# pmelchior/proxmin

Measured on AMD Instinct MI355X. Metric: NMF iterations/sec at Y=16384x16384, K=64, higher is better.
Workload: dtype f16x2r (fp16 split MFMA, fp32 accumulate: the residual from the high x high product + an exact K x K correction, two-term gradients; exact fp32's error class)

## Files before the change

proxmin_amd/csrc/k_gfix.hip:

```cpp
#include "pmx_common.h"

constexpr int GFIX_PARTS = 128;

struct GfixArgs {
    const float* X[2];
    int64_t rows[2];
    int K;
    const float* absmax;
    float* part;
    float* Q;
    float* out[2];
    int ld;
    int want[2];
    const DevStatus* status;
    long long* prof;
};
#define GFIX_STAMP(i) do { if (a.prof != nullptr && blockIdx.x == 0 && blockIdx.y == 0 && threadIdx.x == 0) a.prof[i] = wall_clock64(); } while (0)

typedef _Float16 gf16x8 __attribute__((ext_vector_type(8)));

__device__ __forceinline__ float gfix_scale(const float* absmax, int f, float* red) {
    float m = 0.f;
    for (int i = threadIdx.x; i < 256; i += blockDim.x) m = fmaxf(m, absmax[f * 256 + i]);
#pragma unroll
    for (int o = 32; o > 0; o >>= 1) m = fmaxf(m, __shfl_xor(m, o));
    if ((threadIdx.x & 63) == 0) red[threadIdx.x >> 6] = m;
    __syncthreads();
    float mx = red[0];
    for (int i = 1; i < (int)(blockDim.x >> 6); ++i) mx = fmaxf(mx, red[i]);
    int q = 0;
    (void)frexpf(mx, &q);
    return ldexpf(1.f, mx > 0.f ? 14 - q : 0);
}

template <int KT, int W>
__device__ __forceinline__ void gfix_gram_wave(const GfixArgs& a, int f, float* red) {
    constexpr int K = 32 * KT, TPW = KT * KT / 4, NB = KT == 2 ? 8 : 4;
    const int lane = threadIdx.x & 63, l31 = lane & 31, hi = lane >> 5;
    const int64_t rows = a.rows[f];
    const int64_t per = 16 * ((rows + 16 * GFIX_PARTS - 1) / (16 * GFIX_PARTS));
    const int64_t r0 = (int64_t)blockIdx.x * per, r1 = r0 + per < rows ? r0 + per : rows;
    const float* X = a.X[f] + 32 * 0 + l31;
    f32x16 acc0[TPW], accr[TPW];
#pragma unroll
    for (int t = 0; t < TPW; ++t)
#pragma unroll
        for (int i = 0; i < 16; ++i) { acc0[t][i] = 0.f; accr[t][i] = 0.f; }
// ... 145 lines not shown
        const float* p = a.part + (int64_t)f * GFIX_PARTS * n + (int64_t)(q * 32) * n + e;
        float v[32];
#pragma unroll
        for (int i = 0; i < 32; ++i) v[i] = p[(int64_t)i * n];
#pragma unroll
        for (int i = 0; i < 32; ++i) s += (double)v[i];
    }
    const int base = threadIdx.x & 60;
    double tot = __shfl(s, base);
#pragma unroll
    for (int i = 1; i < 4; ++i) tot += __shfl(s, base + i);
    if (e < n && q == 0) a.Q[(int64_t)f * n + e] = (float)tot;
    GFIX_STAMP(5);
}

template <int KT>
__global__ __launch_bounds__(KT == 4 ? 512 : 256) void k_gfix_apply(GfixArgs a) {
    constexpr int K = 32 * KT, LDQ = K + 8;
    constexpr int NT = KT == 4 ? 512 : 256, NW = NT / 64;
    extern __shared__ _Float16 qpl[];
    __shared__ float red[8];
    if (chain_halted(a.status)) return;
    const int f = blockIdx.y;
    if (!a.want[f]) return;
    const int tid = threadIdx.x, lane = tid & 63, w = tid >> 6, l31 = lane & 31, hi = lane >> 5;
    const int64_t rows = a.rows[f];
    const float* X = a.X[f];
    float* out = a.out[f];
    const int64_t ntask = (rows + 31) / 32 * KT, stride = (int64_t)gridDim.x * NW;
    if ((int64_t)blockIdx.x * NW >= ntask) return;
    GFIX_STAMP(6);
    f32x4 x[K / 16][2];
#define GFIX_LOAD_X(t_)                                                                                                   \
    {                                                                                                                     \
        const int64_t row_ = ((t_) / KT) * 32 + l31;                                                                      \
        const f32x4* xr = reinterpret_cast<const f32x4*>(X + (row_ < rows ? row_ : 0) * K + 8 * hi);                       \
        _Pragma("unroll") for (int ks = 0; ks < K / 16; ++ks) { x[ks][0] = xr[4 * ks]; x[ks][1] = xr[4 * ks + 1]; }       \
    }
    const int64_t task0 = (int64_t)blockIdx.x * NW + w;
    if (task0 < ntask) GFIX_LOAD_X(task0)
    constexpr int TPK = NT / K, NBLK = K / 8 / TPK;
    const int kcol = tid % K, kb0 = tid / K;
    float tq[2][NBLK][8];
    {
        const float* src = a.Q + (int64_t)(1 - f) * 2 * K * K;
#pragma unroll
        for (int m = 0; m < 2; ++m)
#pragma unroll
            for (int i = 0; i < NBLK; ++i)
#pragma unroll
                for (int e = 0; e < 8; ++e) tq[m][i][e] = src[(size_t)m * K * K + (size_t)(8 * (kb0 + TPK * i) + e) * K + kcol];
    }
    float mx[2] = {0.f, 0.f};
#pragma unroll
    for (int m = 0; m < 2; ++m)
// ... 1 lines not shown
        for (int i = 0; i < NBLK; ++i)
#pragma unroll
            for (int e = 0; e < 8; ++e) mx[m] = fmaxf(mx[m], fabsf(tq[m][i][e]));
#pragma unroll
    for (int o = 32; o > 0; o >>= 1) { mx[0] = fmaxf(mx[0], __shfl_xor(mx[0], o)); mx[1] = fmaxf(mx[1], __shfl_xor(mx[1], o)); }
    __shared__ float redq[2][NW];
    if (lane == 0) { redq[0][w] = mx[0]; redq[1][w] = mx[1]; }
    const float sc = gfix_scale(a.absmax, f, red);
    GFIX_STAMP(7);
    float sq[2];
#pragma unroll
    for (int m = 0; m < 2; ++m) {
        float v = redq[m][0];
#pragma unroll
        for (int i = 1; i < NW; ++i) v = fmaxf(v, redq[m][i]);
        int q = 0;
        (void)frexpf(v, &q);
        sq[m] = ldexpf(1.f, v > 0.f ? 14 - q : 0);
    }
#pragma unroll
    for (int m = 0; m < 2; ++m) {
        _Float16* ph = qpl + (size_t)((1 - m) * 2) * K * LDQ + (size_t)kcol * LDQ;
        _Float16* pl = ph + (size_t)K * LDQ;
#pragma unroll
        for (int i = 0; i < NBLK; ++i) {
            gf16x8 h8, l8;
#pragma unroll
            for (int e = 0; e < 8; ++e) {
                const float v = tq[m][i][e] * sq[m];
                const _Float16 h = (_Float16)v;
                h8[e] = h;
                l8[e] = (_Float16)(v - (float)h);
            }
            *reinterpret_cast<gf16x8*>(ph + 8 * (kb0 + TPK * i)) = h8;
            *reinterpret_cast<gf16x8*>(pl + 8 * (kb0 + TPK * i)) = l8;
        }
    }
    __syncthreads();
    GFIX_STAMP(8);
    for (int64_t task = (int64_t)blockIdx.x * NW + w; task < ntask; task += stride) {
        const int64_t rt = task / KT;
        const int c = (int)(task % KT);
        const bool live = rt * 32 + l31 < rows;
        if (task != task0) GFIX_LOAD_X(task)
        f32x16 acc1, acc2;
#pragma unroll
        for (int i = 0; i < 16; ++i) { acc1[i] = 0.f; acc2[i] = 0.f; }
        const _Float16* qb = qpl + (size_t)(32 * c + l31) * LDQ + 8 * hi;
#pragma unroll
        for (int ks = 0; ks < K / 16; ++ks) {
            gf16x8 xh, xl, xm;
#pragma unroll
            for (int e = 0; e < 8; ++e) {
                const float v = (live ? x[ks][e >> 2][e & 3] : 0.f) * sc;
                const _Float16 h = (_Float16)v;
                const float r1 = v - (float)h;
                const _Float16 l = (_Float16)r1;
                xh[e] = h; xl[e] = l; xm[e] = (_Float16)(r1 - (float)l);
            }
            const gf16x8 qrh = *reinterpret_cast<const gf16x8*>(qb + 16 * ks);
            const gf16x8 qrl = *reinterpret_cast<const gf16x8*>(qb + (size_t)K * LDQ + 16 * ks);
            const gf16x8 q0h = *reinterpret_cast<const gf16x8*>(qb + (size_t)2 * K * LDQ + 16 * ks);
            const gf16x8 q0l = *reinterpret_cast<const gf16x8*>(qb + (size_t)3 * K * LDQ + 16 * ks);
            acc1 = __builtin_amdgcn_mfma_f32_32x32x16_f16(xl, qrh, acc1, 0, 0, 0);
            acc2 = __builtin_amdgcn_mfma_f32_32x32x16_f16(xm, q0h, acc2, 0, 0, 0);
            acc1 = __builtin_amdgcn_mfma_f32_32x32x16_f16(xh, qrl, acc1, 0, 0, 0);
            acc2 = __builtin_amdgcn_mfma_f32_32x32x16_f16(xl, q0l, acc2, 0, 0, 0);
            acc1 = __builtin_amdgcn_mfma_f32_32x32x16_f16(xh, qrh, acc1, 0, 0, 0);
            acc2 = __builtin_amdgcn_mfma_f32_32x32x16_f16(xl, q0h, acc2, 0, 0, 0);
        }
        const float u1 = 1.f / (sc * sq[1]), u2 = 1.f / (sc * sq[0]);
#pragma unroll
        for (int i = 0; i < 16; ++i) {
            const int64_t r = rt * 32 + (i & 3) + 8 * (i >> 2) + 4 * hi;
            if (r < rows) out[r * a.ld + 32 * c + l31] = acc1[i] * u1 + acc2[i] * u2;
        }
        GFIX_STAMP(9);
    }
#undef GFIX_LOAD_X
    GFIX_STAMP(10);
}

static hipError_t launch_gfix(const GfixArgs& a, hipStream_t s) {
    const int n = 2 * a.K * a.K;
    const size_t lds = (size_t)4 * a.K * (a.K + 8) * sizeof(_Float16);
    const int64_t rmax = a.rows[0] > a.rows[1] ? a.rows[0] : a.rows[1];
    const int nw = a.K == 128 ? 8 : 4;
    unsigned nb = (unsigned)(((rmax + 31) / 32 * (a.K / 32) + nw - 1) / nw);
    if (nb > (a.K == 128 ? 128u : 256u)) nb = a.K == 128 ? 128 : 256;
    if (a.K == 64) {
        hipError_t e = hipFuncSetAttribute((const void*)k_gfix_apply<2>, hipFuncAttributeMaxDynamicSharedMemorySize, (int)lds);
        if (e != hipSuccess) return e;
        hipLaunchKernelGGL(k_gfix_gram<2>, dim3(GFIX_PARTS, 2), dim3(256), 0, s, a);
        hipLaunchKernelGGL(k_gfix_reduce, dim3((n * 4 + 255) / 256, 2), dim3(256), 0, s, a);
        hipLaunchKernelGGL(k_gfix_apply<2>, dim3(nb, 2), dim3(256), lds, s, a);
    } else if (a.K == 128) {
        hipError_t e = hipFuncSetAttribute((const void*)k_gfix_apply<4>, hipFuncAttributeMaxDynamicSharedMemorySize, (int)lds);
        if (e != hipSuccess) return e;
        e = hipFuncSetAttribute((const void*)k_gfix_gram<4>, hipFuncAttributeMaxDynamicSharedMemorySize, 64 * 1024);
        if (e != hipSuccess) return e;
        hipLaunchKernelGGL(k_gfix_gram<4>, dim3(GFIX_PARTS, 2), dim3(256), 64 * 1024, s, a);
        hipLaunchKernelGGL(k_gfix_reduce, dim3((n * 4 + 255) / 256, 2), dim3(256), 0, s, a);
        hipLaunchKernelGGL(k_gfix_apply<4>, dim3(nb, 2), dim3(512), lds, s, a);
    } else return hipErrorInvalidValue;
    return hipGetLastError();
}
```

proxmin_amd/csrc/k_update.hip:

```cpp
#include "pmx_common.h"

template <int CTRL>
__device__ __forceinline__ float dpp_f(float v) {
    return __builtin_bit_cast(float, __builtin_amdgcn_update_dpp(0, __builtin_bit_cast(int, v), CTRL, 0xf, 0xf, true));
}
template <int CTRL>
__device__ __forceinline__ double dpp_d(double v) {
    const unsigned long long u = __builtin_bit_cast(unsigned long long, v);
    const unsigned lo = (unsigned)__builtin_amdgcn_update_dpp(0, (int)(unsigned)u, CTRL, 0xf, 0xf, true);
    const unsigned hi = (unsigned)__builtin_amdgcn_update_dpp(0, (int)(unsigned)(u >> 32), CTRL, 0xf, 0xf, true);
    return __builtin_bit_cast(double, ((unsigned long long)hi << 32) | lo);
}
constexpr int DPP_XOR1 = 0xB1, DPP_XOR2 = 0x4E, DPP_HALF_MIRROR = 0x141, DPP_MIRROR = 0x140;
constexpr int SWZ_XOR16 = (0x10 << 10) | 0x1f;

constexpr int SWZ_XOR8 = (0x08 << 10) | 0x1f, SWZ_XOR4 = (0x04 << 10) | 0x1f;
__device__ __forceinline__ float row_sum32(float v) {
    v += __builtin_bit_cast(float, __builtin_amdgcn_ds_swizzle(__builtin_bit_cast(int, v), SWZ_XOR16));
    v += __builtin_bit_cast(float, __builtin_amdgcn_ds_swizzle(__builtin_bit_cast(int, v), SWZ_XOR8));
    v += __builtin_bit_cast(float, __builtin_amdgcn_ds_swizzle(__builtin_bit_cast(int, v), SWZ_XOR4));
    v += dpp_f<DPP_XOR2>(v);
    v += dpp_f<DPP_XOR1>(v);
    return v;
}
// ... 1323 lines not shown
        for (unsigned spins = 1; (gb_load(&b->gen[g][0]) >> 1) < e; ++spins) {
            __builtin_amdgcn_s_sleep(4);
            if ((spins & 1023u) == 0 && wall_clock64() - t0 > 10000000) {
                st->tail_fault = 2;
                st->reason = HALT_ERROR;
                __threadfence();
                st->halt = 1;
                break;
            }
        }
    }
    __syncthreads();
}

constexpr int TAIL_NT = 4;
struct TailArgs {
    MomentArgs m;
    ProxSeq prox[2];
    double e_rel[2];
    int prox_max_iter;
    double* colpart;
    float* absmax_out;
    AlphaArgs al;
    int decide_check;
    GridBar* bar;
    int slots[2];
    long long* prof;
    int prof_fine;
};
template <int NC>
__global__ __launch_bounds__(EW_THREADS) void k_ada_tail(TailArgs a) {
    __shared__ double scratch[4 * TAIL_NT * EW_WAVES];
    __shared__ double dbuf[EW_BLOCKS + 8];
    __shared__ unsigned s_word;
    extern __shared__ float lds[];
    static_assert(EW_BLOCKS == 2 * MAXK, "the step-size phase gives one (block, component) to each workgroup");
    DevStatus* st = a.m.status;
    if (chain_halted(st)) return;
    const int tid = threadIdx.x, l32 = tid & 31;
    const int K = a.m.K;
    GridBar* bar = a.bar;
    unsigned ep = bar->epoch[0];
    int nstamp = 0;
    auto stamp = [&]() { if (a.prof != nullptr && blockIdx.x == 0 && tid == 0) a.prof[nstamp++] = wall_clock64(); };
    stamp();
    if (tid == 0) gb_arrive(bar, ep + 1, true);
    const int64_t hw = ((int64_t)blockIdx.x * EW_THREADS + tid) >> 5;
    const int64_t nhw = ((int64_t)EW_BLOCKS * EW_THREADS) >> 5;
    const int nslot = a.slots[0] + a.slots[1];
    float* Lx = lds;
    float* Lz = lds + (size_t)nslot * NC * EW_THREADS;
    float* Lp = lds + (size_t)2 * nslot * NC * EW_THREADS;
    auto slot = [&](int j, int i, int c) { return ((size_t)((j ? a.slots[0] : 0) + i) * NC + c) * EW_THREADS + tid; };
    bool ok[NC];
#pragma unroll
    for (int c = 0; c < NC; ++c) ok[c] = l32 + 32 * c < K;
    const MomentScalars ms = moment_scalars(a.m);
    const bool any_prox = a.m.has_prox[0] || a.m.has_prox[1];

    float g_pre[NC], x_pre[NC];
    const bool pre = a.slots[0] > 0 && hw < a.m.rows[0];
    if (pre) {
        load_grad<NC>(g_pre, ok, a.m.slab[0], a.m.rows[0], K, hw, l32);
#pragma unroll
        for (int c = 0; c < NC; ++c) x_pre[c] = ok[c] ? a.m.X[0][hw * K + l32 + 32 * c] : 0.f;
    }
    float alpha0[NC], alpha1[NC];
#pragma unroll
    for (int c = 0; c < NC; ++c) {
        alpha0[c] = ok[c] ? st->alpha[0][l32 + 32 * c] : 0.f;
        alpha1[c] = ok[c] ? st->alpha[1][l32 + 32 * c] : 0.f;
    }
    const int last_tau0 = st->last_tau[0], last_tau1 = st->last_tau[1];
    {
        if (tid == 0) s_word = gb_wait(bar, ep + 1, 200000);
        __syncthreads();
        if (s_word & 1u) {
            if (blockIdx.x == 0 && tid == 0) {
                st->tail_fault = 1;
                st->reason = HALT_ERROR;
                __threadfence();
                st->halt = 1;
            }
            return;
        }
        ep += 1;
    }
    stamp();
// ... 3 lines not shown
        float alpha[NC];
#pragma unroll
        for (int c = 0; c < NC; ++c) alpha[c] = j ? alpha1[c] : alpha0[c];
        float maxpsi = -1.f;
        for (int i = 0; i < a.slots[j]; ++i) {
            const int64_t r = hw + (int64_t)i * nhw;
            if (r >= rows) break;
            float g[NC], xo[NC];
            if (j == 0 && i == 0 && pre) {
#pragma unroll
                for (int c = 0; c < NC; ++c) { g[c] = g_pre[c]; xo[c] = x_pre[c]; }
            } else {
                load_grad<NC>(g, ok, a.m.slab[j], rows, K, r, l32);
#pragma unroll
                for (int c = 0; c < NC; ++c) xo[c] = ok[c] ? a.m.X[j][r * K + l32 + 32 * c] : 0.f;
            }
#pragma unroll
            for (int c = 0; c < NC; ++c) {
                if (!ok[c]) continue;
                const int64_t e = r * K + l32 + 32 * c;
                float psi;
                const float xn = moment_elem(a.m, ms, j, e, g[c], alpha[c], xo[c], psi);
                if (a.m.check_convergence) a.m.Xp[j][e] = xo[c];
                Lx[slot(j, i, c)] = xn;
                Lp[slot(j, i, c)] = psi;
                maxpsi = nanmaxf(maxpsi, psi);
            }
        }
        if (j) mpsi1 = maxpsi; else mpsi0 = maxpsi;
    }
// ... 861 lines not shown
    do {                                                                                                           \
        if ((K) <= 32) hipLaunchKernelGGL((KERNEL<1, NT>), grid, dim3(EW_THREADS), 0, stream, args);                \
        else if ((K) <= 64) hipLaunchKernelGGL((KERNEL<2, NT>), grid, dim3(EW_THREADS), 0, stream, args);           \
        else hipLaunchKernelGGL((KERNEL<4, NT>), grid, dim3(EW_THREADS), 0, stream, args);                          \
    } while (0)
void launch_ada_sub(const SubArgs& a, hipStream_t s) {
    if (a.nt == 1) DISPATCH_NC_NT(a.K, 1, k_ada_sub, dim3(EW_BLOCKS, 2), s, a);
    else if (a.nt == 4) DISPATCH_NC_NT(a.K, 4, k_ada_sub, dim3(EW_BLOCKS, 2), s, a);
    else DISPATCH_NC_NT(a.K, SUB_NT_MAX, k_ada_sub, dim3(EW_BLOCKS, 2), s, a);
}
void launch_ada_finish(const FinishArgs& a, hipStream_t s) { DISPATCH_NC(a.s.K, k_ada_finish, dim3(EW_BLOCKS, 2), s, a); }
void launch_ada_decide(const AdaDecideArgs& a, hipStream_t s) { hipLaunchKernelGGL(k_ada_decide, dim3(1), dim3(EW_THREADS), 0, s, a); }
static size_t ada_tail_lds_bytes(const TailArgs& a) {
    const int NC = a.m.K <= 32 ? 1 : (a.m.K <= 64 ? 2 : 4);
    const size_t arr = (size_t)(a.slots[0] + a.slots[1]) * NC * EW_THREADS * sizeof(float);
    return 2 * arr + std::max(arr, (size_t)(EW_THREADS / 32) * MAXK * sizeof(float));
}
constexpr size_t ADA_TAIL_LDS_MAX = 160 * 1024 - 6 * 1024;
template <int NC>
static hipError_t launch_ada_tail_t(const TailArgs& a, hipStream_t s) {
    const size_t lds = ada_tail_lds_bytes(a);
    hipError_t e = hipFuncSetAttribute((const void*)k_ada_tail<NC>, hipFuncAttributeMaxDynamicSharedMemorySize, (int)lds);
    if (e != hipSuccess) return e;
    hipLaunchKernelGGL(k_ada_tail<NC>, dim3(EW_BLOCKS), dim3(EW_THREADS), lds, s, a);
    return hipGetLastError();
}
hipError_t launch_ada_tail(const TailArgs& a, hipStream_t s) {
    if (a.m.K <= 32) return launch_ada_tail_t<1>(a, s);
    if (a.m.K <= 64) return launch_ada_tail_t<2>(a, s);
    return launch_ada_tail_t<4>(a, s);
}
// ... 8 lines not shown
```

proxmin_amd/csrc/pmx_api.hip:

```cpp
#include <stdarg.h>
#include <stdio.h>
#include <string.h>
#include <math.h>
#include <vector>
#include <string>
#include <algorithm>
#include <mutex>

#include <fcntl.h>
#include <sys/file.h>
#include <unistd.h>
#include <dlfcn.h>
#include <link.h>
#include "pmx_common.h"
#include "chain_link.h"
#include "k_grad.hip"
#include "k_grad_bf16.hip"
#include "k_grad_k128.hip"
#include "k_grad_f16_k32.hip"
#include "k_grad_f32pc.hip"
#include "k_update.hip"
#include "k_gram.hip"
#include "k_gfix.hip"
#include "k_small_f64.hip"
#include "k_grad_f64.hip"
#include "k_big_f64.hip"

static thread_local char g_err[512] = "";
void pmx_set_error(const char* fmt, ...) {
    va_list ap;
    va_start(ap, fmt);
    vsnprintf(g_err, sizeof(g_err), fmt, ap);
    va_end(ap);
}
#define FAIL(code, ...)            \
    do {                           \
        pmx_set_error(__VA_ARGS__); \
        return (code);             \
// ... 68 lines not shown
    bool use_bf16 = false;
    bool use_f16 = false;
    bool k128 = false;
    bool k32f16 = false;
    bool f32pc = false;
    bool f16_fell_back = false;
    bool f16_scales = false;
    float rangeRatio = 65536.f;
    int rangeFaults = 0;
    int f16_r3 = 0;
    float* fixPart = nullptr;
    float* fixQ = nullptr;
    float* fixSlab[2] = {nullptr, nullptr};
    long long* fixProf = nullptr;
    bool fix_on = false;
    bool k1_sync_check = false;
    int ncu = 0;
    _Float16* A16[2] = {nullptr, nullptr};
    float* absmax = nullptr;
    float ymax = 0.f;
    float wmax = 1.f;
    bool absmax_by_finish = false;
    bool gram_by_update = false;
    bool bsd_decide_pending = false;
    BsdmmDecideArgs bsd_decide{};
    bool gram_fresh[2] = {false, false};
    bool gram_in_update = true;
    bool fold_in_k1 = true;
    K1GramFold k1_fold{};
    bool decide_pending = false;
// ... 457 lines not shown
    }
    for (int a = 0; a < 6; ++a) ms[a] = cnt[a] ? sum[a] / cnt[a] : 0.0;
    *iterations = cnt[0];
    return PMX_OK;
}

extern "C" int pmx_k1_info(pmx_ctx* c, int info[8]) {
    if (!c || !info) FAIL(PMX_E_INVALID, "NULL argument");
    info[0] = c->f64big ? 13 : c->f64 ? 7 : c->k32f16 ? (c->f16_r3 ? 10 : 8) : c->use_small ? 4 : (c->k128 ? (c->f16_r3 == 2 && !c->W && c->fixPart ? 12 : 5) : (c->use_f16 && !c->f16_fell_back ? (c->f16_r3 && !c->W ? (c->f16_r3 == 2 && c->fixPart ? 11 : 9) : 2) : (c->use_bf16 ? 1 : (c->f32pc ? 6 : 0))));
    info[1] = c->chainL;
    info[2] = c->nSlabA;
    info[3] = c->nSlabS;
    info[4] = c->plan.gridX;
    info[5] = c->plan.gridY;
    info[6] = c->plan.RP;
    info[7] = c->chainFaults + 1000 * c->tailFaults + (c->tail_fused ? 1000000 : 0) + 10000000 * std::min(c->rangeFaults, 9);
    return PMX_OK;
}

extern "C" int pmx_k1_frame(pmx_ctx* c, int64_t frame[3]) {
    if (!c || !frame) FAIL(PMX_E_INVALID, "NULL argument");
    frame[0] = c->f64 ? c->M : c->Mk;
    frame[1] = c->f64 ? c->N : c->Nk;
    frame[2] = c->f64 ? c->K : c->Kk;
    return PMX_OK;
}

extern "C" int pmx_ctx_sync(pmx_ctx* c) {
    if (!c) FAIL(PMX_E_INVALID, "ctx is NULL");
    HIP_CHECK(hipStreamSynchronize(c->stream));
    return PMX_OK;
// ... 306 lines not shown
    c->nSlabA = c->plan.nSlabA;
    float* big = nullptr;
    int rc = dallocT(c, &big, (size_t)c->nSlabA * c->Mk * c->Kk, false);
    if (rc != PMX_OK) return rc;
    c->slab[0] = big;
    return PMX_OK;
}
static int one_iteration_per_call(pmx_ctx* c) {
    c->k1_sync_check = true;
    return chain_disable(c);
}
static int k1_leave_f16(pmx_ctx* c) {
    c->mode = PMX_MODE_F32;
    select_k1(c, c->Mk, c->Nk, c->ncu);
    c->fix_on = false;
    if (c->k1_sync_check) {
        c->chainL = 0;
        c->nSlabA = c->plan.nSlabA;
    }
    c->chainFlags = nullptr;
    c->chainSeq = 0;
    c->slab[0] = c->slab[1] = nullptr;
    c->lossPart = nullptr;
    int rc = PMX_OK;
    if (c->chainL > 0) rc = dallocT(c, &c->chainFlags, (size_t)(c->plan.gridX * c->plan.gridY / c->chainL) * c->plan.RP * 4);
    if (rc == PMX_OK) rc = dallocT(c, &c->slab[0], (size_t)c->nSlabA * c->Mk * c->Kk, false);
    if (rc == PMX_OK) rc = dallocT(c, &c->slab[1], (size_t)c->plan.nSlabS * c->Nk * c->Kk, false);
    if (rc == PMX_OK) rc = dallocT(c, &c->lossPart, (size_t)2 * c->plan.gridX * c->plan.gridY);
    c->rangeFaults += 1;
    return rc;
// ... 68 lines not shown
    if (timed) HIP_CHECK(hipEventRecord(c->ev[c->ev_used], c->stream));
    HIP_CHECK(launch_small_front(c->plan, g, e, c->stream));
    c->nloss = c->plan.gridX * c->plan.gridY;
    if (timed) {
        HIP_CHECK(hipEventRecord(c->ev[c->ev_used + 1], c->stream));
        c->ev_used += 2;
    }
    return PMX_OK;
}

static int k1_prio_for(const pmx_ctx* c, int kk) {
    if (c->k1_prio != -999) return c->k1_prio;
    return kk == 64 ? 0 : 1;
}

static int enqueue_gfix(pmx_ctx* c, const float* A, const float* St, int doA, int doS, hipStream_t stream) {
    GfixArgs f{};
    f.X[0] = A; f.X[1] = St;
    f.rows[0] = c->M; f.rows[1] = c->N;
    f.K = (int)c->Kk;
    f.absmax = c->absmax;
    f.part = c->fixPart; f.Q = c->fixQ;
    f.out[0] = c->fixSlab[0]; f.out[1] = c->fixSlab[1];
    f.ld = (int)c->Kk;
    f.want[0] = (doA & 1) != 0; f.want[1] = doS != 0;
    f.status = c->dstatus;
    f.prof = c->fixProf;
    HIP_CHECK(launch_gfix(f, stream));
    return PMX_OK;
}

static int enqueue_grad_once(pmx_ctx* c, const float* A, const float* St, int doA, int doS, bool absmax_fresh) {
    if (c->host_grad) return PMX_OK;
    if (c->Kk != c->K) {
        PadArgs pa{};
        pa.src[0] = A; pa.src[1] = St;
        pa.dst[0] = c->Xk[0]; pa.dst[1] = c->Xk[1];
        pa.rows[0] = c->M; pa.rows[1] = c->N;
        pa.K = (int)c->K; pa.Kk = (int)c->Kk;
        pa.status = c->dstatus;
        launch_pad_factors(pa, c->stream);
        A = c->Xk[0]; St = c->Xk[1];
    }
    const int64_t Kq = c->Kk;
    bool fix_pending = false;
    const bool timed = c->timing && (c->timing_seq++ % (unsigned)c->timing_stride) == 0 && c->ev_used + 2 <= c->ev.size();
    if (c->k128) {
// ... 110 lines not shown
                HIP_CHECK(hipMemsetAsync(c->chainFlags, 0, (size_t)(c->plan.gridX * c->plan.gridY / c->chainL) * c->plan.RP * 4 * sizeof(unsigned), c->stream));
                c->chainSeq = 0;
            }
            GradArgs gc = g;
            gc.chainL = c->chainL; gc.chainFlags = c->chainFlags; gc.chainBase = (++c->chainSeq) * 64u; gc.wstatus = c->dstatus;
            gc.chainInject = c->hook_inject_k1 > 0 && (int)c->chainSeq == c->hook_inject_k1;
            HIP_CHECK(grad_launch_f32pc(c->plan, gc, c->stream));
        } else
        HIP_CHECK(c->use_small ? grad_launch_small(c->plan, g, c->stream) : (c->f32pc ? grad_launch_f32pc(c->plan, g, c->stream) : grad_launch_f32(c->plan, g, c->stream)));
        c->nloss = c->plan.gridX * c->plan.gridY;
    }
    if (timed) {
        HIP_CHECK(hipEventRecord(c->ev[c->ev_used + 1], c->stream));
        c->ev_used += 2;
    }
    if ((doA & 1) || doS) c->fix_on = fix_pending;
    if (fix_pending) { const int rcf = enqueue_gfix(c, A, St, doA, doS, c->stream); if (rcf != PMX_OK) return rcf; }
    return PMX_OK;
}

static int enqueue_grad(pmx_ctx* c, const float* A, const float* St, int doA, int doS, bool absmax_fresh = false) {
    int rc = enqueue_grad_once(c, A, St, doA, doS, absmax_fresh);
    if (rc != PMX_OK || !c->k1_sync_check || !c->f16_scales || c->host_grad || !(doA | doS)) return rc;
    rc = read_status(c);
    if (rc != PMX_OK) return rc;
    if (c->hstatus->k1_fault != 4) return PMX_OK;
    int again = 0;
    rc = chain_fault_fallback(c, &again);
    if (rc != PMX_OK) return rc;
    return enqueue_grad_once(c, A, St, doA, doS, false);
}

static SlabRef slab_ref(pmx_ctx* c, int j) {
    SlabRef s;
    s.stride = c->rowsK[j] * c->Kk;
    s.ld = (int)c->Kk;
    if (c->host_grad) {
        s.base = c->G[j];
        s.n = 1;
        s.ld = (int)c->K;
        return s;
    }
    s.base = c->slab[j];
    s.n = j == 0 ? c->nSlabA : c->nSlabS;
    if (c->fix_on) s.extra = c->fixSlab[j];
// ... 1283 lines not shown
        m.slab[1].base = c->ssplit ? c->comm_out : c->comm;
        m.slab[1].n = 1; m.slab[1].ld = (int)c->K; m.slab[1].extra = nullptr;
    }
    m.K = (int)c->K;
    m.status = c->dstatus;
    m.partials = c->partials;
    m.scheme = p.scheme;
    m.it = it;
    m.b1t = b1t; m.b1prev = b1prev; m.b2 = p.b2; m.eps = p.eps; m.p = p.p;
    m.check_convergence = p.check_convergence;
    launch_ada_moment(m, c->stream);
    HIP_CHECK(hipGetLastError());
    return PMX_OK;
}

static int ada_enqueue_tail_fused(pmx_ctx* c, int it, double b1t, double b1prev) {
    const pmx_adaprox_params& p = c->ada;
    TailArgs t{};
    MomentArgs& m = t.m;
    for (int j = 0; j < 2; ++j) {
        m.X[j] = s_view(c, j, c->X[j]); m.Xp[j] = s_view(c, j, c->Xp[j]);
        m.Mm[j] = s_view(c, j, c->Mm[j]); m.Vv[j] = s_view(c, j, c->Vv[j]);
        m.Vh[j] = p.warm_vhat ? s_view(c, j, c->Vh[j]) : nullptr;
        m.Psi[j] = nullptr;
        m.slab[j] = slab_ref(c, j);
        m.rows[j] = upd_rows(c, j);
        m.has_prox[j] = p.prox[j].n > 0;
        t.prox[j] = to_dev(p.prox[j]);
        t.e_rel[j] = p.e_rel[j];
        t.slots[j] = (int)((upd_rows(c, j) + 8191) / 8192);
// ... 5 lines not shown
    m.scheme = p.scheme;
    m.it = it;
    m.b1t = b1t; m.b1prev = b1prev; m.b2 = p.b2; m.eps = p.eps; m.p = p.p;
    m.check_convergence = p.check_convergence;
    t.prox_max_iter = p.prox_max_iter;
    t.colpart = c->colpart;
    t.absmax_out = c->f16_scales ? c->absmax : nullptr;
    t.al = alpha_args(c);
    t.al.use_fixed = p.use_fixed_steps;
    t.al.fixed[0] = (float)p.fixed_alpha[0];
    t.al.fixed[1] = (float)p.fixed_alpha[1];
    t.decide_check = c->comm ? 0 : 1;
    t.bar = c->gridbar;
    t.prof = c->tailprof;
    t.prof_fine = getenv("PMX_TAIL_PROF") && atoi(getenv("PMX_TAIL_PROF")) == 2;
    const char* lockfile = c->hook_tail_lockfile.empty() ? nullptr : c->hook_tail_lockfile.c_str();
    int lockfd = -1;
    if (lockfile) {
        lockfd = open(lockfile, O_CREAT | O_RDWR, 0600);
        if (lockfd < 0) FAIL(PMX_E_STATE, "PMX_TAIL_LOCKFILE: cannot open %s", lockfile);
        HIP_CHECK(hipStreamSynchronize(c->stream));
        if (flock(lockfd, LOCK_EX) != 0) { close(lockfd); FAIL(PMX_E_STATE, "PMX_TAIL_LOCKFILE: flock failed"); }
    }
    hipError_t le = launch_ada_tail(t, c->stream);
    if (lockfd >= 0) {
        hipError_t se = hipStreamSynchronize(c->stream);
        flock(lockfd, LOCK_UN);
        close(lockfd);
        HIP_CHECK(se);
    }
// ... 123 lines not shown
            if (rc != PMX_OK) return rc;
            if (c->hstatus->halt && c->hstatus->reason == HALT_ERROR) FAIL(PMX_E_HIP, "%s", chain_error_text(c));
        }
        fill_result(c, res, it0);
        return PMX_OK;
    }
    int done = 0;
    int tails = 0;
    while (done < n_iter && !c->hstatus->stopped) {
        const int chunk = std::min(n_iter - done, c->tail_fused ? 64 : 16);
        const int nsub = any_prox ? std::max(1, std::min(c->nsub_guess, p.prox_max_iter)) : 0;
        if (c->sub_nt != 1) c->sub_nt = nsub <= 4 ? 4 : SUB_NT_MAX;
        for (int i = 0; i < chunk; ++i) {
            const int gi = done + i;
            if (c->tail_fused) {
                rc = enqueue_grad(c, c->X[0], c->X[1], 1, 1, tails > 0);
                if (rc == PMX_OK) rc = ada_enqueue_tail_fused(c, it0 + gi, b1[gi], gi == 0 ? b1_prev : b1[gi - 1]);
                ++tails;
                if (rc != PMX_OK) return rc;
                continue;
            }
            rc = ada_enqueue_head(c, it0 + gi, b1[gi], gi == 0 ? b1_prev : b1[gi - 1], tails > 0);
            if (rc != PMX_OK) return rc;
            rc = ada_enqueue_tail(c, ada_enqueue_subs(c, 0, nsub));
            ++tails;
            if (rc != PMX_OK) return rc;
        }
        rc = read_status(c);
        if (rc != PMX_OK) return rc;
        const int nsub_enq = nsub > 0 ? ((nsub + c->sub_nt - 1) / c->sub_nt) * c->sub_nt : 0;
        int t_enq = nsub_enq;
// ... 17 lines not shown
            if (c->hstatus->it_done > it_before) t_enq = nsub_enq;
        }
        done = c->hstatus->it_done - it0;
        {
            int again = 0;
            rc = chain_fault_fallback(c, &again);
            if (rc != PMX_OK) return rc;
            if (again) { tails = 0; continue; }
        }
        if (any_prox) c->nsub_guess = std::max(2, std::max(c->hstatus->last_tau[0], c->hstatus->last_tau[1]));
        if (c->hstatus->halt && c->hstatus->reason == HALT_ERROR) FAIL(PMX_E_HIP, "%s", chain_error_text(c));
    }
    if (c->tailprof && c->tail_fused) {
        long long h[16];
        HIP_CHECK(hipMemcpy(h, c->tailprof, sizeof(h), hipMemcpyDeviceToHost));
        static const char* nm[] = {"census", "moment", "B1", "maxpsi", "sub", "B2", "judge+replay", "finish", "B3", "decide"};
        static const char* nf[] = {"census", "moment", "B1", "maxpsi", "passesA", "sumsA", "passesS", "sumsS", "(end)", "B2", "judge+replay", "finish", "B3", "decide"};
        const bool fine = getenv("PMX_TAIL_PROF") && atoi(getenv("PMX_TAIL_PROF")) == 2;
        const int np = fine ? 14 : 10;
        fprintf(stderr, "[tailprof] us:");
        for (int i = 0; i < np; ++i) fprintf(stderr, " %s=%.2f", fine ? nf[i] : nm[i], (double)(h[i + 1] - h[i]) / 100.0);
        fprintf(stderr, " total=%.2f\n", (double)(h[np] - h[0]) / 100.0);
    }
    fill_result(c, res, it0);
    return PMX_OK;
}

extern "C" int pmx_adaprox_set_alpha(pmx_ctx* c, const float* alpha) {
    REJECT_F64(c);
    if (!c || !alpha) FAIL(PMX_E_INVALID, "NULL argument");
    if (c->algo != ALG_ADAPROX || c->ada.use_fixed_steps != 2) FAIL(PMX_E_STATE, "pmx_adaprox_begin with use_fixed_steps = 2 has not been called");
    HIP_CHECK(hipSetDevice(c->device));
    HIP_CHECK(hipMemcpyAsync(&c->dstatus->alpha[0][0], alpha, sizeof(float) * c->K, hipMemcpyHostToDevice, c->stream));
    HIP_CHECK(hipMemcpyAsync(&c->dstatus->alpha[1][0], alpha + c->K, sizeof(float) * c->K, hipMemcpyHostToDevice, c->stream));
// ... 837 lines not shown
```

proxmin_amd/engine.py:

```python
from __future__ import annotations

import ctypes as C
import logging
import os

import numpy as np

from . import _lib

logger = logging.getLogger("proxmin")
_noticed = set()


def _notice(key, msg):
    if key not in _noticed:
        _noticed.add(key)
        logger.info(msg)


LIBRARY_DEFAULT_MODE = "f16x2r"
_DEFAULT_MODE = os.environ.get("PMX_MODE", LIBRARY_DEFAULT_MODE)
assert _DEFAULT_MODE in ("f32", "bf16x3", "f16x2", "f16x2r"), "PMX_MODE must be one of f32, bf16x3, f16x2, f16x2r"


# ... 226 lines not shown
        return {k: ms[i] for i, k in enumerate(self.PHASES)}, n.value

    def time_grad(self, do_A=True, do_S=True, reps=10):
        ms = C.c_double()
        _lib.check(self.lib.pmx_time_grad(self.h, int(do_A), int(do_S), int(reps), C.byref(ms)))
        return ms.value

    def k1_info(self):
        v = (C.c_int * 8)()
        _lib.check(self.lib.pmx_k1_info(self.h, v))
        keys = ("kernel", "chain", "slabs_A", "slabs_S", "row_regions", "col_regions", "panels_per_region", "chain_faults")
        d = dict(zip(keys, list(v)))
        d["kernel"] = ("k_grad_f32", "k_grad_bf16", "k_grad_f16_v8", "k_grad_f16_v9", "k_grad_small", "k_grad_f16_k128", "k_grad_f32_pc", "k64_front", "k_grad_f16_k32", "k_grad_f16_v8_r3", "k_grad_f16_k32_r3", "k_grad_f16_v8_hh", "k_grad_f16_k128_hh", "k64_grad_pass")[d["kernel"]]
        v7 = d.pop("chain_faults")
        d["chain_faults"], d["tail_faults"], d["tail_fused"] = v7 % 1000, (v7 // 1000) % 1000, bool((v7 // 1000000) % 10)
        d["range_faults"] = v7 // 10000000
        fr = (C.c_int64 * 3)()
        _lib.check(self.lib.pmx_k1_frame(self.h, fr))
        d["frame"] = (fr[0], fr[1])
        d["frame_K"] = fr[2]
        return d

    def grad(self):
        _lib.check(self.lib.pmx_grad(self.h))
        return self._download(_lib.BUF_GA, self.M), self._download(_lib.BUF_GST, self.N).T

    def loglike(self):
        out = C.c_double()
        _lib.check(self.lib.pmx_loglike(self.h, C.byref(out)))
        return out.value

# ... 143 lines not shown
```

Before: 2797.

## Fuse gradient K×K correction apply into the fused Adaprox tail kernel

For K=64 with the fused tail path, the separate k_gfix_apply launch is skipped. The tail kernel now builds the fp16 hi/lo correction planes in LDS, computes the correction tiles with MFMA for each slot, and adds them to the gradient before the update. This removes one kernel launch and the write and re-read of the corrected gradient through global memory. In exchange the tail kernel needs more LDS and does extra MFMA work before its grid barrier arrive, which can delay the barrier. Shared apply code is factored into helpers reused by both kernels.

```diff
diff --git a/proxmin_amd/csrc/k_gfix.hip b/proxmin_amd/csrc/k_gfix.hip
--- a/proxmin_amd/csrc/k_gfix.hip
+++ b/proxmin_amd/csrc/k_gfix.hip
@@ -19,6 +19,12 @@
 
 typedef _Float16 gf16x8 __attribute__((ext_vector_type(8)));
 
+__device__ __forceinline__ float gfix_pow2(float m) {
+    int q = 0;
+    (void)frexpf(m, &q);
+    return ldexpf(1.f, m > 0.f ? 14 - q : 0);
+}
+
 __device__ __forceinline__ float gfix_scale(const float* absmax, int f, float* red) {
     float m = 0.f;
     for (int i = threadIdx.x; i < 256; i += blockDim.x) m = fmaxf(m, absmax[f * 256 + i]);
@@ -28,9 +34,7 @@
     __syncthreads();
     float mx = red[0];
     for (int i = 1; i < (int)(blockDim.x >> 6); ++i) mx = fmaxf(mx, red[i]);
-    int q = 0;
-    (void)frexpf(mx, &q);
-    return ldexpf(1.f, mx > 0.f ? 14 - q : 0);
+    return gfix_pow2(mx);
 }
 
 template <int KT, int W>
@@ -206,6 +210,53 @@
     GFIX_STAMP(5);
 }
 
+template <int K>
+__device__ __forceinline__ void gfix_load_row(f32x4 (&x)[K / 16][2], const float* X, int64_t row, int64_t rows, int hi) {
+    const f32x4* xr = reinterpret_cast<const f32x4*>(X + (row < rows ? row : 0) * K + 8 * hi);
+#pragma unroll
+    for (int ks = 0; ks < K / 16; ++ks) { x[ks][0] = xr[4 * ks]; x[ks][1] = xr[4 * ks + 1]; }
+}
+__device__ __forceinline__ void gfix_split8(const float (&v)[8], float s, gf16x8& h8, gf16x8& l8) {
+#pragma unroll
+    for (int e = 0; e < 8; ++e) {
+        const float t = v[e] * s;
+        const _Float16 h = (_Float16)t;
+        h8[e] = h;
+        l8[e] = (_Float16)(t - (float)h);
+    }
+}
+template <int K, int LDQ>
+__device__ __forceinline__ void gfix_apply_tile(const f32x4 (&x)[K / 16][2], bool live, float sc, const _Float16* qb, f32x16& acc1, f32x16& acc2) {
+#pragma unroll
+    for (int i = 0; i < 16; ++i) { acc1[i] = 0.f; acc2[i] = 0.f; }
+#pragma unroll
+    for (int ks = 0; ks < K / 16; ++ks) {
+        gf16x8 xh, xl, xm;
+#pragma unroll
+        for (int e = 0; e < 8; ++e) {
+            const float v = (live ? x[ks][e >> 2][e & 3] : 0.f) * sc;
+            const _Float16 h = (_Float16)v;
+            const float r1 = v - (float)h;
+            const _Float16 l = (_Float16)r1;
+            xh[e] = h; xl[e] = l; xm[e] = (_Float16)(r1 - (float)l);
+        }
+        const gf16x8 qrh = *reinterpret_cast<const gf16x8*>(qb + 16 * ks);
+        const gf16x8 qrl = *reinterpret_cast<const gf16x8*>(qb + (size_t)K * LDQ + 16 * ks);
+        const gf16x8 q0h = *reinterpret_cast<const gf16x8*>(qb + (size_t)2 * K * LDQ + 16 * ks);
+        const gf16x8 q0l = *reinterpret_cast<const gf16x8*>(qb + (size_t)3 * K * LDQ + 16 * ks);
+        acc1 = __builtin_amdgcn_mfma_f32_32x32x16_f16(xl, qrh, acc1, 0, 0, 0);
+        acc2 = __builtin_amdgcn_mfma_f32_32x32x16_f16(xm, q0h, acc2, 0, 0, 0);
+        acc1 = __builtin_amdgcn_mfma_f32_32x32x16_f16(xh, qrl, acc1, 0, 0, 0);
+        acc2 = __builtin_amdgcn_mfma_f32_32x32x16_f16(xl, q0l, acc2, 0, 0, 0);
+        acc1 = __builtin_amdgcn_mfma_f32_32x32x16_f16(xh, qrh, acc1, 0, 0, 0);
+        acc2 = __builtin_amdgcn_mfma_f32_32x32x16_f16(xl, q0h, acc2, 0, 0, 0);
+    }
+}
+__device__ __forceinline__ float gfix_combine(float a1, float u1, float a2, float u2) {
+#pragma clang fp contract(off)
+    return a1 * u1 + a2 * u2;
+}
+
 template <int KT>
 __global__ __launch_bounds__(KT == 4 ? 512 : 256) void k_gfix_apply(GfixArgs a) {
     constexpr int K = 32 * KT, LDQ = K + 8;
@@ -223,14 +274,8 @@
     if ((int64_t)blockIdx.x * NW >= ntask) return;
     GFIX_STAMP(6);
     f32x4 x[K / 16][2];
-#define GFIX_LOAD_X(t_)                                                                                                   \
-    {                                                                                                                     \
-        const int64_t row_ = ((t_) / KT) * 32 + l31;                                                                      \
-        const f32x4* xr = reinterpret_cast<const f32x4*>(X + (row_ < rows ? row_ : 0) * K + 8 * hi);                       \
-        _Pragma("unroll") for (int ks = 0; ks < K / 16; ++ks) { x[ks][0] = xr[4 * ks]; x[ks][1] = xr[4 * ks + 1]; }       \
-    }
     const int64_t task0 = (int64_t)blockIdx.x * NW + w;
-    if (task0 < ntask) GFIX_LOAD_X(task0)
+    if (task0 < ntask) gfix_load_row<K>(x, X, (task0 / KT) * 32 + l31, rows, hi);
     constexpr int TPK = NT / K, NBLK = K / 8 / TPK;
     const int kcol = tid % K, kb0 = tid / K;
     float tq[2][NBLK][8];
@@ -262,9 +307,7 @@
         float v = redq[m][0];
 #pragma unroll
         for (int i = 1; i < NW; ++i) v = fmaxf(v, redq[m][i]);
-        int q = 0;
-        (void)frexpf(v, &q);
-        sq[m] = ldexpf(1.f, v > 0.f ? 14 - q : 0);
+        sq[m] = gfix_pow2(v);
     }
 #pragma unroll
     for (int m = 0; m < 2; ++m) {
@@ -273,13 +316,7 @@
 #pragma unroll
         for (int i = 0; i < NBLK; ++i) {
             gf16x8 h8, l8;
-#pragma unroll
-            for (int e = 0; e < 8; ++e) {
-                const float v = tq[m][i][e] * sq[m];
-                const _Float16 h = (_Float16)v;
-                h8[e] = h;
-                l8[e] = (_Float16)(v - (float)h);
-            }
+            gfix_split8(tq[m][i], sq[m], h8, l8);
             *reinterpret_cast<gf16x8*>(ph + 8 * (kb0 + TPK * i)) = h8;
             *reinterpret_cast<gf16x8*>(pl + 8 * (kb0 + TPK * i)) = l8;
         }
@@ -290,46 +327,21 @@
         const int64_t rt = task / KT;
         const int c = (int)(task % KT);
         const bool live = rt * 32 + l31 < rows;
-        if (task != task0) GFIX_LOAD_X(task)
+        if (task != task0) gfix_load_row<K>(x, X, rt * 32 + l31, rows, hi);
         f32x16 acc1, acc2;
-#pragma unroll
-        for (int i = 0; i < 16; ++i) { acc1[i] = 0.f; acc2[i] = 0.f; }
-        const _Float16* qb = qpl + (size_t)(32 * c + l31) * LDQ + 8 * hi;
-#pragma unroll
-        for (int ks = 0; ks < K / 16; ++ks) {
-            gf16x8 xh, xl, xm;
-#pragma unroll
-            for (int e = 0; e < 8; ++e) {
-                const float v = (live ? x[ks][e >> 2][e & 3] : 0.f) * sc;
-                const _Float16 h = (_Float16)v;
-                const float r1 = v - (float)h;
-                const _Float16 l = (_Float16)r1;
-                xh[e] = h; xl[e] = l; xm[e] = (_Float16)(r1 - (float)l);
-            }
-            const gf16x8 qrh = *reinterpret_cast<const gf16x8*>(qb + 16 * ks);
-            const gf16x8 qrl = *reinterpret_cast<const gf16x8*>(qb + (size_t)K * LDQ + 16 * ks);
-            const gf16x8 q0h = *reinterpret_cast<const gf16x8*>(qb + (size_t)2 * K * LDQ + 16 * ks);
-            const gf16x8 q0l = *reinterpret_cast<const gf16x8*>(qb + (size_t)3 * K * LDQ + 16 * ks);
-            acc1 = __builtin_amdgcn_mfma_f32_32x32x16_f16(xl, qrh, acc1, 0, 0, 0);
-            acc2 = __builtin_amdgcn_mfma_f32_32x32x16_f16(xm, q0h, acc2, 0, 0, 0);
-            acc1 = __builtin_amdgcn_mfma_f32_32x32x16_f16(xh, qrl, acc1, 0, 0, 0);
-            acc2 = __builtin_amdgcn_mfma_f32_32x32x16_f16(xl, q0l, acc2, 0, 0, 0);
-            acc1 = __builtin_amdgcn_mfma_f32_32x32x16_f16(xh, qrh, acc1, 0, 0, 0);
-            acc2 = __builtin_amdgcn_mfma_f32_32x32x16_f16(xl, q0h, acc2, 0, 0, 0);
-        }
+        gfix_apply_tile<K, LDQ>(x, live, sc, qpl + (size_t)(32 * c + l31) * LDQ + 8 * hi, acc1, acc2);
         const float u1 = 1.f / (sc * sq[1]), u2 = 1.f / (sc * sq[0]);
 #pragma unroll
         for (int i = 0; i < 16; ++i) {
             const int64_t r = rt * 32 + (i & 3) + 8 * (i >> 2) + 4 * hi;
-            if (r < rows) out[r * a.ld + 32 * c + l31] = acc1[i] * u1 + acc2[i] * u2;
+            if (r < rows) out[r * a.ld + 32 * c + l31] = gfix_combine(acc1[i], u1, acc2[i], u2);
         }
         GFIX_STAMP(9);
     }
-#undef GFIX_LOAD_X
     GFIX_STAMP(10);
 }
 
-static hipError_t launch_gfix(const GfixArgs& a, hipStream_t s) {
+static hipError_t launch_gfix(const GfixArgs& a, hipStream_t s, bool apply = true) {
     const int n = 2 * a.K * a.K;
     const size_t lds = (size_t)4 * a.K * (a.K + 8) * sizeof(_Float16);
     const int64_t rmax = a.rows[0] > a.rows[1] ? a.rows[0] : a.rows[1];
@@ -341,8 +353,8 @@
         if (e != hipSuccess) return e;
         hipLaunchKernelGGL(k_gfix_gram<2>, dim3(GFIX_PARTS, 2), dim3(256), 0, s, a);
         hipLaunchKernelGGL(k_gfix_reduce, dim3((n * 4 + 255) / 256, 2), dim3(256), 0, s, a);
-        hipLaunchKernelGGL(k_gfix_apply<2>, dim3(nb, 2), dim3(256), lds, s, a);
-    } else if (a.K == 128) {
+        if (apply) hipLaunchKernelGGL(k_gfix_apply<2>, dim3(nb, 2), dim3(256), lds, s, a);
+    } else if (a.K == 128 && apply) {
         hipError_t e = hipFuncSetAttribute((const void*)k_gfix_apply<4>, hipFuncAttributeMaxDynamicSharedMemorySize, (int)lds);
         if (e != hipSuccess) return e;
         e = hipFuncSetAttribute((const void*)k_gfix_gram<4>, hipFuncAttributeMaxDynamicSharedMemorySize, 64 * 1024);
diff --git a/proxmin_amd/csrc/k_update.hip b/proxmin_amd/csrc/k_update.hip
--- a/proxmin_amd/csrc/k_update.hip
+++ b/proxmin_amd/csrc/k_update.hip
@@ -1361,6 +1361,12 @@
 }
 
 constexpr int TAIL_NT = 4;
+constexpr int TAIL_FIX_K = 64, TAIL_FIX_LDQ = TAIL_FIX_K + 8;
+constexpr size_t TAIL_FIX_PLANES = (size_t)2 * 4 * TAIL_FIX_K * TAIL_FIX_LDQ * sizeof(_Float16);
+struct TailFix {
+    const float* Q;
+    const float* absmax;
+};
 struct TailArgs {
     MomentArgs m;
     ProxSeq prox[2];
@@ -1374,6 +1380,7 @@
     int slots[2];
     long long* prof;
     int prof_fine;
+    TailFix fix;
 };
 template <int NC>
 __global__ __launch_bounds__(EW_THREADS) void k_ada_tail(TailArgs a) {
@@ -1391,7 +1398,8 @@
     int nstamp = 0;
     auto stamp = [&]() { if (a.prof != nullptr && blockIdx.x == 0 && tid == 0) a.prof[nstamp++] = wall_clock64(); };
     stamp();
-    if (tid == 0) gb_arrive(bar, ep + 1, true);
+    const bool fixing = NC == 2 && a.fix.Q != nullptr;
+    if (tid == 0 && !fixing) gb_arrive(bar, ep + 1, true);
     const int64_t hw = ((int64_t)blockIdx.x * EW_THREADS + tid) >> 5;
     const int64_t nhw = ((int64_t)EW_BLOCKS * EW_THREADS) >> 5;
     const int nslot = a.slots[0] + a.slots[1];
@@ -1405,6 +1413,81 @@
     const MomentScalars ms = moment_scalars(a.m);
     const bool any_prox = a.m.has_prox[0] || a.m.has_prox[1];
 
+    if constexpr (NC == 2) if (fixing) {
+        constexpr int FK = TAIL_FIX_K, LDQ = TAIL_FIX_LDQ;
+        __shared__ float s_fmax[3][EW_WAVES];
+        const int lane = tid & 63, w = tid >> 6, l31 = lane & 31, hi = lane >> 5;
+        const int f = tid >> 9, kcol = tid & (FK - 1), kb = (tid >> 6) & 7;
+        float tq[2][8];
+        {
+            const float* src = a.fix.Q + (size_t)(1 - f) * 2 * FK * FK;
+#pragma unroll
+            for (int m = 0; m < 2; ++m)
+#pragma unroll
+                for (int e = 0; e < 8; ++e) tq[m][e] = src[(size_t)m * FK * FK + (size_t)(8 * kb + e) * FK + kcol];
+        }
+        float am = tid < 2 * 256 ? a.fix.absmax[tid] : 0.f;
+        const int ntask = 2 * nslot;
+        auto task_tile = [&](int task, int& j, int& i) {
+            const int sl = task >> 1;
+            j = sl >= a.slots[0];
+            i = sl - (j ? a.slots[0] : 0);
+            return (int64_t)i * nhw + 32 * (int64_t)blockIdx.x;
+        };
+        f32x4 x[FK / 16][2];
+        if (w < ntask) {
+            int j, i;
+            const int64_t r0 = task_tile(w, j, i);
+            gfix_load_row<FK>(x, a.m.X[j], r0 + l31, a.m.rows[j], hi);
+        }
+        float mq[2] = {0.f, 0.f};
+#pragma unroll
+        for (int m = 0; m < 2; ++m)
+#pragma unroll
+            for (int e = 0; e < 8; ++e) mq[m] = fmaxf(mq[m], fabsf(tq[m][e]));
+#pragma unroll
+        for (int o = 32; o > 0; o >>= 1) {
+            am = fmaxf(am, __shfl_xor(am, o));
+            mq[0] = fmaxf(mq[0], __shfl_xor(mq[0], o));
+            mq[1] = fmaxf(mq[1], __shfl_xor(mq[1], o));
+        }
+        if (lane == 0) { s_fmax[0][w] = am; s_fmax[1][w] = mq[0]; s_fmax[2][w] = mq[1]; }
+        __syncthreads();
+        if (tid == 0) gb_arrive(bar, ep + 1, true);
+        float sc[2], sq[2][2];
+#pragma unroll
+        for (int b = 0; b < 2; ++b) {
+            float v = s_fmax[0][4 * b], v0 = s_fmax[1][8 * b], v1 = s_fmax[2][8 * b];
+            for (int q = 1; q < 4; ++q) v = fmaxf(v, s_fmax[0][4 * b + q]);
+            for (int q = 1; q < 8; ++q) { v0 = fmaxf(v0, s_fmax[1][8 * b + q]); v1 = fmaxf(v1, s_fmax[2][8 * b + q]); }
+            sc[b] = gfix_pow2(v);
+            sq[b][0] = gfix_pow2(v0);
+            sq[b][1] = gfix_pow2(v1);
+        }
+        _Float16* planes = reinterpret_cast<_Float16*>(Lp);
+#pragma unroll
+        for (int m = 0; m < 2; ++m) {
+            _Float16* ph = planes + (size_t)(f * 4 + (1 - m) * 2) * FK * LDQ + (size_t)kcol * LDQ + 8 * kb;
+            gf16x8 h8, l8;
+            gfix_split8(tq[m], sq[f][m], h8, l8);
+            *reinterpret_cast<gf16x8*>(ph) = h8;
+            *reinterpret_cast<gf16x8*>(ph + (size_t)FK * LDQ) = l8;
+        }
+        __syncthreads();
+        for (int task = w; task < ntask; task += EW_WAVES) {
+            int j, i;
+            const int64_t r0 = task_tile(task, j, i);
+            if (r0 >= a.m.rows[j]) continue;
+            if (task != w) gfix_load_row<FK>(x, a.m.X[j], r0 + l31, a.m.rows[j], hi);
+            const int c = task & 1;
+            f32x16 acc1, acc2;
+            gfix_apply_tile<FK, LDQ>(x, r0 + l31 < a.m.rows[j], sc[j], planes + (size_t)(j * 4) * FK * LDQ + (size_t)(32 * c + l31) * LDQ + 8 * hi, acc1, acc2);
+            const float u1 = 1.f / (sc[j] * sq[j][1]), u2 = 1.f / (sc[j] * sq[j][0]);
+            float* dst = Lz + ((size_t)((j ? a.slots[0] : 0) + i) * NC + c) * EW_THREADS + l31;
+#pragma unroll
+            for (int q = 0; q < 16; ++q) dst[32 * ((q & 3) + 8 * (q >> 2) + 4 * hi)] = gfix_combine(acc1[q], u1, acc2[q], u2);
+        }
+    }
     float g_pre[NC], x_pre[NC];
     const bool pre = a.slots[0] > 0 && hw < a.m.rows[0];
     if (pre) {
@@ -1419,6 +1502,8 @@
         alpha1[c] = ok[c] ? st->alpha[1][l32 + 32 * c] : 0.f;
     }
     const int last_tau0 = st->last_tau[0], last_tau1 = st->last_tau[1];
+
+    stamp();
     {
         if (tid == 0) s_word = gb_wait(bar, ep + 1, 200000);
         __syncthreads();
@@ -1452,6 +1537,11 @@
                 load_grad<NC>(g, ok, a.m.slab[j], rows, K, r, l32);
 #pragma unroll
                 for (int c = 0; c < NC; ++c) xo[c] = ok[c] ? a.m.X[j][r * K + l32 + 32 * c] : 0.f;
+            }
+            if (fixing) {
+#pragma unroll
+                for (int c = 0; c < NC; ++c)
+                    if (ok[c]) g[c] += Lz[slot(j, i, c)];
             }
 #pragma unroll
             for (int c = 0; c < NC; ++c) {
@@ -2343,7 +2433,8 @@
 static size_t ada_tail_lds_bytes(const TailArgs& a) {
     const int NC = a.m.K <= 32 ? 1 : (a.m.K <= 64 ? 2 : 4);
     const size_t arr = (size_t)(a.slots[0] + a.slots[1]) * NC * EW_THREADS * sizeof(float);
-    return 2 * arr + std::max(arr, (size_t)(EW_THREADS / 32) * MAXK * sizeof(float));
+    const size_t base = 2 * arr + std::max(arr, (size_t)(EW_THREADS / 32) * MAXK * sizeof(float));
+    return a.fix.Q != nullptr ? std::max(base, 2 * arr + TAIL_FIX_PLANES) : base;
 }
 constexpr size_t ADA_TAIL_LDS_MAX = 160 * 1024 - 6 * 1024;
 template <int NC>
diff --git a/proxmin_amd/csrc/pmx_api.hip b/proxmin_amd/csrc/pmx_api.hip
--- a/proxmin_amd/csrc/pmx_api.hip
+++ b/proxmin_amd/csrc/pmx_api.hip
@@ -19,9 +19,9 @@
 #include "k_grad_k128.hip"
 #include "k_grad_f16_k32.hip"
 #include "k_grad_f32pc.hip"
+#include "k_gfix.hip"
 #include "k_update.hip"
 #include "k_gram.hip"
-#include "k_gfix.hip"
 #include "k_small_f64.hip"
 #include "k_grad_f64.hip"
 #include "k_big_f64.hip"
@@ -120,6 +120,8 @@
     float* fixSlab[2] = {nullptr, nullptr};
     long long* fixProf = nullptr;
     bool fix_on = false;
+    bool fix_tail = false;
+    bool fix_tail_used = false;
     bool k1_sync_check = false;
     int ncu = 0;
     _Float16* A16[2] = {nullptr, nullptr};
@@ -607,7 +609,7 @@
     info[4] = c->plan.gridX;
     info[5] = c->plan.gridY;
     info[6] = c->plan.RP;
-    info[7] = c->chainFaults + 1000 * c->tailFaults + (c->tail_fused ? 1000000 : 0) + 10000000 * std::min(c->rangeFaults, 9);
+    info[7] = c->chainFaults + 1000 * c->tailFaults + (c->tail_fused ? 1000000 : 0) + 10000000 * std::min(c->rangeFaults, 9) + (c->fix_tail_used ? 100000000 : 0);
     return PMX_OK;
 }
 
@@ -944,6 +946,7 @@
     c->mode = PMX_MODE_F32;
     select_k1(c, c->Mk, c->Nk, c->ncu);
     c->fix_on = false;
+    c->fix_tail = false;
     if (c->k1_sync_check) {
         c->chainL = 0;
         c->nSlabA = c->plan.nSlabA;
@@ -1042,7 +1045,7 @@
     return kk == 64 ? 0 : 1;
 }
 
-static int enqueue_gfix(pmx_ctx* c, const float* A, const float* St, int doA, int doS, hipStream_t stream) {
+static int enqueue_gfix(pmx_ctx* c, const float* A, const float* St, int doA, int doS, hipStream_t stream, bool apply) {
     GfixArgs f{};
     f.X[0] = A; f.X[1] = St;
     f.rows[0] = c->M; f.rows[1] = c->N;
@@ -1054,11 +1057,11 @@
     f.want[0] = (doA & 1) != 0; f.want[1] = doS != 0;
     f.status = c->dstatus;
     f.prof = c->fixProf;
-    HIP_CHECK(launch_gfix(f, stream));
-    return PMX_OK;
-}
-
-static int enqueue_grad_once(pmx_ctx* c, const float* A, const float* St, int doA, int doS, bool absmax_fresh) {
+    HIP_CHECK(launch_gfix(f, stream, apply));
+    return PMX_OK;
+}
+
+static int enqueue_grad_once(pmx_ctx* c, const float* A, const float* St, int doA, int doS, bool absmax_fresh, bool tail_fix) {
     if (c->host_grad) return PMX_OK;
     if (c->Kk != c->K) {
         PadArgs pa{};
@@ -1199,13 +1202,14 @@
         HIP_CHECK(hipEventRecord(c->ev[c->ev_used + 1], c->stream));
         c->ev_used += 2;
     }
-    if ((doA & 1) || doS) c->fix_on = fix_pending;
-    if (fix_pending) { const int rcf = enqueue_gfix(c, A, St, doA, doS, c->stream); if (rcf != PMX_OK) return rcf; }
-    return PMX_OK;
-}
-
-static int enqueue_grad(pmx_ctx* c, const float* A, const float* St, int doA, int doS, bool absmax_fresh = false) {
-    int rc = enqueue_grad_once(c, A, St, doA, doS, absmax_fresh);
+    const bool in_tail = fix_pending && tail_fix && (doA & 1) && doS && Kq == TAIL_FIX_K && c->K == Kq;
+    if ((doA & 1) || doS) { c->fix_on = fix_pending && !in_tail; c->fix_tail = in_tail; }
+    if (fix_pending) { const int rcf = enqueue_gfix(c, A, St, doA, doS, c->stream, !in_tail); if (rcf != PMX_OK) return rcf; }
+    return PMX_OK;
+}
+
+static int enqueue_grad(pmx_ctx* c, const float* A, const float* St, int doA, int doS, bool absmax_fresh = false, bool tail_fix = false) {
+    int rc = enqueue_grad_once(c, A, St, doA, doS, absmax_fresh, tail_fix);
     if (rc != PMX_OK || !c->k1_sync_check || !c->f16_scales || c->host_grad || !(doA | doS)) return rc;
     rc = read_status(c);
     if (rc != PMX_OK) return rc;
@@ -1213,7 +1217,7 @@
     int again = 0;
     rc = chain_fault_fallback(c, &again);
     if (rc != PMX_OK) return rc;
-    return enqueue_grad_once(c, A, St, doA, doS, false);
+    return enqueue_grad_once(c, A, St, doA, doS, false, tail_fix);
 }
 
 static SlabRef slab_ref(pmx_ctx* c, int j) {
@@ -2527,6 +2531,15 @@
     return PMX_OK;
 }
 
+static bool ada_tail_can_fix(pmx_ctx* c) {
+    if (!c->tail_fused || c->comm != nullptr || c->shard_grad_from_comm || c->host_grad || c->K != TAIL_FIX_K || c->Kk != TAIL_FIX_K) return false;
+    TailArgs probe{};
+    probe.m.K = (int)c->K;
+    for (int j = 0; j < 2; ++j) probe.slots[j] = (int)((upd_rows(c, j) + 8191) / 8192);
+    probe.fix.Q = c->fixQ;
+    return c->fixQ != nullptr && ada_tail_lds_bytes(probe) <= ADA_TAIL_LDS_MAX;
+}
+
 static int ada_enqueue_tail_fused(pmx_ctx* c, int it, double b1t, double b1prev) {
     const pmx_adaprox_params& p = c->ada;
     TailArgs t{};
@@ -2562,6 +2575,11 @@
     t.bar = c->gridbar;
     t.prof = c->tailprof;
     t.prof_fine = getenv("PMX_TAIL_PROF") && atoi(getenv("PMX_TAIL_PROF")) == 2;
+    if (c->fix_tail && c->comm == nullptr) {
+        t.fix.Q = c->fixQ;
+        t.fix.absmax = c->absmax;
+        c->fix_tail_used = true;
+    }
     const char* lockfile = c->hook_tail_lockfile.empty() ? nullptr : c->hook_tail_lockfile.c_str();
     int lockfd = -1;
     if (lockfile) {
@@ -2715,7 +2733,7 @@
         for (int i = 0; i < chunk; ++i) {
             const int gi = done + i;
             if (c->tail_fused) {
-                rc = enqueue_grad(c, c->X[0], c->X[1], 1, 1, tails > 0);
+                rc = enqueue_grad(c, c->X[0], c->X[1], 1, 1, tails > 0, ada_tail_can_fix(c));
                 if (rc == PMX_OK) rc = ada_enqueue_tail_fused(c, it0 + gi, b1[gi], gi == 0 ? b1_prev : b1[gi - 1]);
                 ++tails;
                 if (rc != PMX_OK) return rc;
@@ -2763,10 +2781,10 @@
     if (c->tailprof && c->tail_fused) {
         long long h[16];
         HIP_CHECK(hipMemcpy(h, c->tailprof, sizeof(h), hipMemcpyDeviceToHost));
-        static const char* nm[] = {"census", "moment", "B1", "maxpsi", "sub", "B2", "judge+replay", "finish", "B3", "decide"};
-        static const char* nf[] = {"census", "moment", "B1", "maxpsi", "passesA", "sumsA", "passesS", "sumsS", "(end)", "B2", "judge+replay", "finish", "B3", "decide"};
+        static const char* nm[] = {"correction", "census", "moment", "B1", "maxpsi", "sub", "B2", "judge+replay", "finish", "B3", "decide"};
+        static const char* nf[] = {"correction", "census", "moment", "B1", "maxpsi", "passesA", "sumsA", "passesS", "sumsS", "(end)", "B2", "judge+replay", "finish", "B3", "decide"};
         const bool fine = getenv("PMX_TAIL_PROF") && atoi(getenv("PMX_TAIL_PROF")) == 2;
-        const int np = fine ? 14 : 10;
+        const int np = fine ? 15 : 11;
         fprintf(stderr, "[tailprof] us:");
         for (int i = 0; i < np; ++i) fprintf(stderr, " %s=%.2f", fine ? nf[i] : nm[i], (double)(h[i + 1] - h[i]) / 100.0);
         fprintf(stderr, " total=%.2f\n", (double)(h[np] - h[0]) / 100.0);
diff --git a/proxmin_amd/engine.py b/proxmin_amd/engine.py
--- a/proxmin_amd/engine.py
+++ b/proxmin_amd/engine.py
@@ -264,7 +264,8 @@
         d["kernel"] = ("k_grad_f32", "k_grad_bf16", "k_grad_f16_v8", "k_grad_f16_v9", "k_grad_small", "k_grad_f16_k128", "k_grad_f32_pc", "k64_front", "k_grad_f16_k32", "k_grad_f16_v8_r3", "k_grad_f16_k32_r3", "k_grad_f16_v8_hh", "k_grad_f16_k128_hh", "k64_grad_pass")[d["kernel"]]
         v7 = d.pop("chain_faults")
         d["chain_faults"], d["tail_faults"], d["tail_fused"] = v7 % 1000, (v7 // 1000) % 1000, bool((v7 // 1000000) % 10)
-        d["range_faults"] = v7 // 10000000
+        d["range_faults"] = (v7 // 10000000) % 10
+        d["tail_fix"] = bool((v7 // 100000000) % 10)
         fr = (C.c_int64 * 3)()
         _lib.check(self.lib.pmx_k1_frame(self.h, fr))
         d["frame"] = (fr[0], fr[1])
```

Result: faster. 2842, median of 6 (+1.6%).
